# adaly/gridnext

Hardware: AMD Instinct MI355X
Metric: spots/sec training throughput (multimodal f+g) (higher is better)
Workload: dtype f32; 1 GPU; C4: multimodal f(DenseNet-121 @128px + count-MLP 2000 genes) + hex g on 78x64 Visium grids, 1 array (4992 spots) per GPU per step, f frozen/eval (tutorial mode), g trained with Adam, masked CE; spots_per_array=4992, parallelism=dp1

## Files before the change

gridnext_amd/csrc/stem_pool.hip:

```cpp
#include <type_traits>
#include "fwd_common.h"

namespace {

__global__ __launch_bounds__(256) void u8_to_f32_kernel(const uint8_t* __restrict__ x8, float* __restrict__ out, long n4,
                                                        long hw4, int C, const float* __restrict__ nrm) {
    const long stride = (long)gridDim.x * blockDim.x;
    for (long i = (long)blockIdx.x * blockDim.x + threadIdx.x; i < n4; i += stride) {
        const int c = (int)((i / hw4) % C);
        const bool norm = nrm != nullptr && c < 3;
        const float mean = norm ? nrm[c] : 0.f, sd = norm ? nrm[3 + c] : 1.f, rsd = norm ? nrm[6 + c] : 1.f;
        const uint32_t wv = reinterpret_cast<const uint32_t*>(x8)[i];
        reinterpret_cast<float4*>(out)[i] = u8x4_pixels(wv, norm, mean, sd, rsd);
    }
}

constexpr int ST_BM = 128, ST_BN = 64;

__global__ __launch_bounds__(256) void conv_stem_kernel(const float* __restrict__ x, const float* __restrict__ w,
                                                        float* __restrict__ out, long ldc, long M, int Cin, int H,
                                                        int Wd, int Ho, int Wo, int O, int KH, int KW, int stride,
                                                        int pad) {
    extern __shared__ __attribute__((aligned(16))) float lds[];
    const int KC = KH * 8, LD = KC + 4;
// ... 11 lines not shown
#pragma unroll
    for (int p = 0; p < 4; ++p) {
        const long row = m0 + rr + 32 * p;
        rok[p] = row < M;
        const long img = row / ((long)Ho * Wo);
        const int rem = (int)(row - img * Ho * Wo);
        const int oy = rem / Wo, ox = rem - oy * Wo;
        ibase[p] = img * Cin * (long)H * Wd;
        iy0[p] = oy * stride - pad;
        ix0[p] = ox * stride - pad + kx;
    }
    f32x16 acc[2];
#pragma unroll
    for (int a = 0; a < 2; ++a)
#pragma unroll
        for (int r = 0; r < 16; ++r) acc[a][r] = 0.f;

    for (int c = 0; c < Cin; ++c) {
        __syncthreads();
#pragma unroll
        for (int p = 0; p < 4; ++p) {
            const bool xok = rok[p] && kx < KW && ix0[p] >= 0 && ix0[p] < Wd;
            const float* xc = x + ibase[p] + (long)c * H * Wd;
            for (int ky = 0; ky < KH; ++ky) {
                const int iy = iy0[p] + ky;
                float v = 0.f;
                if (xok && iy >= 0 && iy < H) v = xc[(long)iy * Wd + ix0[p]];
                As[(rr + 32 * p) * LD + ky * 8 + kx] = v;
            }
        }
#pragma unroll
        for (int p = 0; p < 2; ++p) {
            const int o = n0 + rr + 32 * p;
            for (int ky = 0; ky < KH; ++ky) {
                float v = 0.f;
                if (o < O && kx < KW) v = w[(((long)o * Cin + c) * KH + ky) * KW + kx];
                Bs[(rr + 32 * p) * LD + ky * 8 + kx] = v;
            }
        }
        __syncthreads();
        for (int s = 0; s < KH; ++s) {
            const float4 a0 = ld4(&As[(64 * wm + i) * LD + 8 * s + 4 * h]);
            const float4 a1 = ld4(&As[(64 * wm + 32 + i) * LD + 8 * s + 4 * h]);
            const float4 b = ld4(&Bs[(32 * wn + i) * LD + 8 * s + 4 * h]);
            acc[0] = __builtin_amdgcn_mfma_f32_32x32x2f32(a0.x, b.x, acc[0], 0, 0, 0);
            acc[1] = __builtin_amdgcn_mfma_f32_32x32x2f32(a1.x, b.x, acc[1], 0, 0, 0);
            acc[0] = __builtin_amdgcn_mfma_f32_32x32x2f32(a0.y, b.y, acc[0], 0, 0, 0);
            acc[1] = __builtin_amdgcn_mfma_f32_32x32x2f32(a1.y, b.y, acc[1], 0, 0, 0);
            acc[0] = __builtin_amdgcn_mfma_f32_32x32x2f32(a0.z, b.z, acc[0], 0, 0, 0);
            acc[1] = __builtin_amdgcn_mfma_f32_32x32x2f32(a1.z, b.z, acc[1], 0, 0, 0);
            acc[0] = __builtin_amdgcn_mfma_f32_32x32x2f32(a0.w, b.w, acc[0], 0, 0, 0);
            acc[1] = __builtin_amdgcn_mfma_f32_32x32x2f32(a1.w, b.w, acc[1], 0, 0, 0);
        }
    }
    const int col = n0 + 32 * wn + i;
    if (col < O) {
#pragma unroll
        for (int mt = 0; mt < 2; ++mt)
#pragma unroll
            for (int r = 0; r < 16; ++r) {
                const long row = m0 + 64 * wm + 32 * mt + (r & 3) + 8 * (r >> 2) + 4 * h;
                if (row < M) out[row * ldc + col] = acc[mt][r];
            }
    }
}

template <int STRIDE, int KH, int CIN>
__global__ __launch_bounds__(256) void conv_stem_patch_kernel(const float* __restrict__ x, const float* __restrict__ w,
                                                              float* __restrict__ out, long ldc, int Cin, int H, int Wd,
                                                              int Ho, int Wo, int O, int KW, int pad, int tiles_x,
                                                              int tiles_y, long ntiles) {
    extern __shared__ __attribute__((aligned(16))) float lds[];
    constexpr int PH = 7 * STRIDE + KH, PW = (15 * STRIDE + 8 + 1) & ~1;
    const int KT = Cin * KH * 8, LDB = KT + 4;
    float* Bs = lds;
    float* Ps = lds + 64 * LDB;
    const int t = threadIdx.x, lane = t & 63, wave = t >> 6, h = lane >> 5, i = lane & 31;
    for (int idx = t; idx < 64 * KT; idx += 256) {
        const int n = idx / KT, rem = idx - n * KT;
        const int kx = rem & 7, cky = rem >> 3;
        float v = 0.f;
        if (n < O && kx < KW) v = w[((long)n * Cin * KH + cky) * KW + kx];
        Bs[n * LDB + rem] = v;
    }
    const int trow = 32 * wave + i;
    const int oyl = trow >> 4, oxl = trow & 15;
    const float* pa = Ps + (STRIDE * oyl) * PW + STRIDE * oxl + 4 * h;
    const float* pb = Bs + i * LDB + 4 * h;

    for (long tile = blockIdx.x; tile < ntiles; tile += gridDim.x) {
        const long img = tile / ((long)tiles_x * tiles_y);
        const int trem = (int)(tile - img * tiles_x * tiles_y);
        const int ty = trem / tiles_x, tx = trem - ty * tiles_x;
        const int oy0 = ty * 8, ox0 = tx * 16;
        const int iy0 = oy0 * STRIDE - pad, ix0 = ox0 * STRIDE - pad;
        __syncthreads();
        for (int idx = t; idx < Cin * PH * PW; idx += 256) {
            const int px = idx % PW, py = (idx / PW) % PH, c = idx / (PW * PH);
            const int iy = iy0 + py, ix = ix0 + px;
            float v = 0.f;
            if (iy >= 0 && iy < H && ix >= 0 && ix < Wd) v = x[((img * Cin + c) * H + iy) * (long)Wd + ix];
            Ps[idx] = v;
        }
        __syncthreads();
        f32x16 acc0, acc1;
#pragma unroll
        for (int r = 0; r < 16; ++r) { acc0[r] = 0.f; acc1[r] = 0.f; }
        auto load_a = [&](int step) {
            const float* ap = pa + ((step / KH) * PH + (step % KH)) * PW;
            if (STRIDE % 2 == 0) {
                const float2 lo = *reinterpret_cast<const float2*>(ap);
                const float2 hi = *reinterpret_cast<const float2*>(ap + 2);
                return make_float4(lo.x, lo.y, hi.x, hi.y);
            }
            return make_float4(ap[0], ap[1], ap[2], ap[3]);
        };
        constexpr int NSTEP = CIN * KH;
        float4 a = load_a(0), b0 = ld4(pb), b1 = ld4(pb + 32 * LDB);
#pragma unroll
        for (int step = 0; step < NSTEP; ++step) {
            float4 na = a, nb0 = b0, nb1 = b1;
            if (step + 1 < NSTEP) {
                na = load_a(step + 1);
                nb0 = ld4(pb + (step + 1) * 8);
                nb1 = ld4(pb + 32 * LDB + (step + 1) * 8);
            }
            acc0 = __builtin_amdgcn_mfma_f32_32x32x2f32(a.x, b0.x, acc0, 0, 0, 0);
            acc1 = __builtin_amdgcn_mfma_f32_32x32x2f32(a.x, b1.x, acc1, 0, 0, 0);
            acc0 = __builtin_amdgcn_mfma_f32_32x32x2f32(a.y, b0.y, acc0, 0, 0, 0);
            acc1 = __builtin_amdgcn_mfma_f32_32x32x2f32(a.y, b1.y, acc1, 0, 0, 0);
            acc0 = __builtin_amdgcn_mfma_f32_32x32x2f32(a.z, b0.z, acc0, 0, 0, 0);
            acc1 = __builtin_amdgcn_mfma_f32_32x32x2f32(a.z, b1.z, acc1, 0, 0, 0);
            acc0 = __builtin_amdgcn_mfma_f32_32x32x2f32(a.w, b0.w, acc0, 0, 0, 0);
            acc1 = __builtin_amdgcn_mfma_f32_32x32x2f32(a.w, b1.w, acc1, 0, 0, 0);
            a = na; b0 = nb0; b1 = nb1;
            __builtin_amdgcn_sched_group_barrier(0x100, STRIDE % 2 == 0 ? 4 : 6, 0);
            __builtin_amdgcn_sched_group_barrier(0x008, 8, 0);
        }
#pragma unroll
        for (int r = 0; r < 16; ++r) {
            const int rr = 32 * wave + (r & 3) + 8 * (r >> 2) + 4 * h;
            const int oy = oy0 + (rr >> 4), ox = ox0 + (rr & 15);
            if (oy < Ho && ox < Wo) {
                float* o = out + ((img * Ho + oy) * (long)Wo + ox) * ldc;
                if (i < O) o[i] = acc0[r];
                if (32 + i < O) o[32 + i] = acc1[r];
            }
        }
    }
}

constexpr int SP_LDT = 40;
constexpr int SP_LDTH = 72;
template <int WO, bool H16 = false, bool U8 = false, bool IDX = false>
__global__ __launch_bounds__(256) void conv_stem_pool_kernel(const void* __restrict__ xv, const float* __restrict__ w,
                                                             float* __restrict__ out, long ldo, int H, int Wd, int O,
                                                             const float* __restrict__ scale,
                                                             const float* __restrict__ shift, long imgs,
                                                             const float* __restrict__ nrm,
                                                             unsigned char* __restrict__ amax = nullptr,
                                                             const int* __restrict__ src_idx = nullptr, long src_imgs = 0) {
    const float* __restrict__ x = reinterpret_cast<const float*>(xv);
    const uint8_t* __restrict__ x8 = reinterpret_cast<const uint8_t*>(xv);
    constexpr int CIN = 3, KH = 7, KW = 7, STRIDE = 2, PAD = 3;
    constexpr int RT = 128 / WO;
    constexpr int PH = STRIDE * (RT - 1) + KH, PW = ((WO - 1) * STRIDE + 8 + 1 + 1) & ~1;
    constexpr int F4R = WO * STRIDE / 4;
    constexpr int NPC = CIN * PH * F4R, NPRE = (NPC + 255) / 256;
    constexpr int NIT = (WO / 2) * 8 / 256;
    constexpr int KT = CIN * KH * 8, LDB = KT + 4;
    extern __shared__ __attribute__((aligned(16))) float lds[];
    auto store4 = [](float* o, long off, const float4& v) {
        if constexpr (H16) {
            typedef _Float16 half4 __attribute__((ext_vector_type(4)));
            const half4 hv = {(_Float16)v.x, (_Float16)v.y, (_Float16)v.z, (_Float16)v.w};
            *reinterpret_cast<half4*>(reinterpret_cast<_Float16*>(o) + off) = hv;
        } else {
            *reinterpret_cast<float4*>(o + off) = v;
        }
    };
    float* Bs = lds;
    float* Ps = lds + 64 * LDB;
    float* Ts = Ps + CIN * PH * PW;
    const int t = threadIdx.x, lane = t & 63, wave = t >> 6, h = lane >> 5, i = lane & 31;
    for (int idx = t; idx < 64 * KT; idx += 256) {
        const int n = idx / KT, rem = idx - n * KT;
        const int kx = rem & 7, cky = rem >> 3;
        float v = 0.f;
        if (n < O && kx < KW) v = w[((long)n * CIN * KH + cky) * KW + kx];
        Bs[n * LDB + rem] = v;
    }
    for (int idx = t; idx < CIN * PH * PW; idx += 256) Ps[idx] = 0.f;
    const int trow = 32 * wave + i;
    const float* pa = Ps + (STRIDE * (trow / WO)) * PW + STRIDE * (trow % WO) + 4 * h;
    const float* pb = Bs + i * LDB + 4 * h;
    const float sc0 = i < O ? scale[i] : 0.f, sh0 = i < O ? shift[i] : 0.f;
    const float sc1 = 32 + i < O ? scale[32 + i] : 0.f, sh1 = 32 + i < O ? shift[32 + i] : 0.f;
    const int c4 = t & 7, pxa = t >> 3;
    const int Ho2 = (H + 2 * PAD - KH) / STRIDE + 1;
    const int ntt = Ho2 / RT;

    float4 pre[U8 ? 1 : NPRE];
    uint32_t pre8[U8 ? NPRE : 1];
    bool in8[U8 ? NPRE : 1];
    auto fetch_patch = [&](long img, int tt) {
        const int iy0 = RT * tt * STRIDE - PAD;
#pragma unroll
        for (int q = 0; q < NPRE; ++q) {
            const int j = t + 256 * q;
            const int f4 = j % F4R, py = (j / F4R) % PH, c = (j / F4R) / PH;
            const int iy = iy0 + py;
            const bool inside = j < NPC && iy >= 0 && iy < H;
            if constexpr (U8) {
                pre8[q] = 0u;
                in8[q] = inside;
                if (inside)
                    pre8[q] = *reinterpret_cast<const uint32_t*>(x8 + ((img * CIN + c) * H + iy) * (long)Wd + 4 * f4);
            } else {
                pre[q] = make_float4(0.f, 0.f, 0.f, 0.f);
                if (inside) pre[q] = ld4(x + ((img * CIN + c) * H + iy) * (long)Wd + 4 * f4);
            }
        }
    };
    auto stash_patch = [&]() {
#pragma unroll
        for (int q = 0; q < NPRE; ++q) {
            const int j = t + 256 * q;
            if (j < NPC) {
                float* d = Ps + (j / F4R) * PW + PAD + 4 * (j % F4R);
                if constexpr (U8) {
                    const int c = (j / F4R) / PH;
                    const bool norm = nrm != nullptr;
                    const float4 v = in8[q] ? u8x4_pixels(pre8[q], norm, norm ? nrm[c] : 0.f, norm ? nrm[3 + c] : 1.f,
                                                          norm ? nrm[6 + c] : 1.f)
                                            : make_float4(0.f, 0.f, 0.f, 0.f);
                    d[0] = v.x; d[1] = v.y; d[2] = v.z; d[3] = v.w;
                } else {
                    d[0] = pre[q].x; d[1] = pre[q].y; d[2] = pre[q].z; d[3] = pre[q].w;
                }
            }
        }
    };
    auto src_of = [&](long img) -> long {
        if (src_idx == nullptr) return img;
        const long s = src_idx[img];
        return s < 0 ? 0 : (s < src_imgs ? s : src_imgs - 1);
    };
    __syncthreads();
    fetch_patch(src_of(blockIdx.x), 0);

    for (long img = blockIdx.x; img < imgs; img += gridDim.x) {
        const long src = src_of(img);
        float4 carry[2][NIT], carry2[2][NIT];
        unsigned cidx[2][NIT], cidx2[2][NIT];
        const float c0v = IDX ? -1.f : 0.f;
#pragma unroll
        for (int q = 0; q < NIT; ++q) {
            carry[0][q] = carry[1][q] = carry2[0][q] = carry2[1][q] = make_float4(c0v, c0v, c0v, c0v);
            cidx[0][q] = cidx[1][q] = cidx2[0][q] = cidx2[1][q] = 0u;
        }
        for (int tt = 0; tt < ntt; ++tt) {
            __syncthreads();
            stash_patch();
            {
                long nsrc = src;
                int nt2 = tt + 1;
                if (nt2 == ntt) {
                    nt2 = 0;
                    long nimg = img + gridDim.x;
                    if (nimg >= imgs) nimg = blockIdx.x;
                    nsrc = src_of(nimg);
                }
                fetch_patch(nsrc, nt2);
            }
            asm volatile("" ::: "memory");
            __syncthreads();
            f32x16 acc0, acc1;
#pragma unroll
            for (int r = 0; r < 16; ++r) { acc0[r] = 0.f; acc1[r] = 0.f; }
            auto load_a = [&](int step) {
                const float* ap = pa + ((step / KH) * PH + (step % KH)) * PW;
                const float2 lo = *reinterpret_cast<const float2*>(ap);
                const float2 hi = *reinterpret_cast<const float2*>(ap + 2);
                return make_float4(lo.x, lo.y, hi.x, hi.y);
            };
            constexpr int NSTEP = CIN * KH;
            float4 a = load_a(0), b0 = ld4(pb), b1 = ld4(pb + 32 * LDB);
#pragma unroll
            for (int step = 0; step < NSTEP; ++step) {
                float4 na = a, nb0 = b0, nb1 = b1;
                if (step + 1 < NSTEP) {
                    na = load_a(step + 1);
                    nb0 = ld4(pb + (step + 1) * 8);
                    nb1 = ld4(pb + 32 * LDB + (step + 1) * 8);
                }
                acc0 = __builtin_amdgcn_mfma_f32_32x32x2f32(a.x, b0.x, acc0, 0, 0, 0);
                acc1 = __builtin_amdgcn_mfma_f32_32x32x2f32(a.x, b1.x, acc1, 0, 0, 0);
                acc0 = __builtin_amdgcn_mfma_f32_32x32x2f32(a.y, b0.y, acc0, 0, 0, 0);
                acc1 = __builtin_amdgcn_mfma_f32_32x32x2f32(a.y, b1.y, acc1, 0, 0, 0);
                acc0 = __builtin_amdgcn_mfma_f32_32x32x2f32(a.z, b0.z, acc0, 0, 0, 0);
                acc1 = __builtin_amdgcn_mfma_f32_32x32x2f32(a.z, b1.z, acc1, 0, 0, 0);
                acc0 = __builtin_amdgcn_mfma_f32_32x32x2f32(a.w, b0.w, acc0, 0, 0, 0);
                acc1 = __builtin_amdgcn_mfma_f32_32x32x2f32(a.w, b1.w, acc1, 0, 0, 0);
                a = na; b0 = nb0; b1 = nb1;
                __builtin_amdgcn_sched_group_barrier(0x100, 4, 0);
                __builtin_amdgcn_sched_group_barrier(0x008, 8, 0);
            }
#pragma unroll
            for (int pass = 0; pass < 2; ++pass) {
                if (pass == 1) __syncthreads();
#pragma unroll
                for (int r = 0; r < 16; ++r) {
                    const int rr = 32 * wave + (r & 3) + 8 * (r >> 2) + 4 * h;
                    Ts[rr * SP_LDT + i] = pass == 0 ? fmaxf(fmaf(acc0[r], sc0, sh0), 0.f) : fmaxf(fmaf(acc1[r], sc1, sh1), 0.f);
                }
                __syncthreads();
                const int ch = 32 * pass + 4 * c4;
#pragma unroll
                for (int q = 0; q < NIT; ++q) {
                    const int px = pxa + 32 * q;
                    float4 m0 = make_float4(c0v, c0v, c0v, c0v), m1 = m0;
                    unsigned h0 = 0u, h1 = 0u;
                    auto hmax = [](float4& m, unsigned& hx, const float4& v, unsigned col) {
                        if (IDX) {
                            if (v.x > m.x) { m.x = v.x; hx = (hx & 0xffffff00u) | col; }
                            if (v.y > m.y) { m.y = v.y; hx = (hx & 0xffff00ffu) | (col << 8); }
                            if (v.z > m.z) { m.z = v.z; hx = (hx & 0xff00ffffu) | (col << 16); }
                            if (v.w > m.w) { m.w = v.w; hx = (hx & 0x00ffffffu) | (col << 24); }
                        } else {
                            m = make_float4(fmaxf(m.x, v.x), fmaxf(m.y, v.y), fmaxf(m.z, v.z), fmaxf(m.w, v.w));
                        }
                    };
#pragma unroll
                    for (int dx = -1; dx <= 1; ++dx) {
                        const int ox = 2 * px + dx;
                        if (ox < 0) continue;
                        hmax(m0, h0, ld4(&Ts[ox * SP_LDT + 4 * c4]), (unsigned)(dx + 1));
                        if (RT == 2) hmax(m1, h1, ld4(&Ts[(WO + ox) * SP_LDT + 4 * c4]), (unsigned)(dx + 1));
                    }
                    auto vmax = [](const float4& ra, unsigned ia, const float4& rb, unsigned ib, const float4& rc, unsigned ic,
                                   float4& o4, unsigned& oi) {
                        if (IDX) {
                            o4 = ra; oi = ia;
                            const unsigned jb = ib + 0x03030303u, jc = ic + 0x06060606u;
                            if (rb.x > o4.x) { o4.x = rb.x; oi = (oi & 0xffffff00u) | (jb & 0x000000ffu); }
                            if (rb.y > o4.y) { o4.y = rb.y; oi = (oi & 0xffff00ffu) | (jb & 0x0000ff00u); }
                            if (rb.z > o4.z) { o4.z = rb.z; oi = (oi & 0xff00ffffu) | (jb & 0x00ff0000u); }
                            if (rb.w > o4.w) { o4.w = rb.w; oi = (oi & 0x00ffffffu) | (jb & 0xff000000u); }
                            if (rc.x > o4.x) { o4.x = rc.x; oi = (oi & 0xffffff00u) | (jc & 0x000000ffu); }
                            if (rc.y > o4.y) { o4.y = rc.y; oi = (oi & 0xffff00ffu) | (jc & 0x0000ff00u); }
                            if (rc.z > o4.z) { o4.z = rc.z; oi = (oi & 0xff00ffffu) | (jc & 0x00ff0000u); }
                            if (rc.w > o4.w) { o4.w = rc.w; oi = (oi & 0x00ffffffu) | (jc & 0xff000000u); }
                        } else {
                            o4 = make_float4(fmaxf(fmaxf(ra.x, rb.x), rc.x), fmaxf(fmaxf(ra.y, rb.y), rc.y),
                                             fmaxf(fmaxf(ra.z, rb.z), rc.z), fmaxf(fmaxf(ra.w, rb.w), rc.w));
                        }
                    };
                    if (RT == 2) {
                        float4 o4;
                        unsigned oi = 0u;
                        vmax(carry[pass][q], cidx[pass][q], m0, h0, m1, h1, o4, oi);
                        carry[pass][q] = m1;
                        cidx[pass][q] = h1;
                        if (ch < O) {
                            const long prow = (img * (Ho2 / 2) + tt) * (long)(WO / 2) + px;
                            store4(out, prow * ldo + ch, o4);
                            if (IDX) *reinterpret_cast<unsigned*>(amax + prow * O + ch) = oi;
                        }
                    } else {
                        if (tt & 1) {
                            float4 o4;
                            unsigned oi = 0u;
                            vmax(carry2[pass][q], cidx2[pass][q], carry[pass][q], cidx[pass][q], m0, h0, o4, oi);
                            if (ch < O) {
                                const long prow = (img * (Ho2 / 2) + (tt >> 1)) * (long)(WO / 2) + px;
                                store4(out, prow * ldo + ch, o4);
                                if (IDX) *reinterpret_cast<unsigned*>(amax + prow * O + ch) = oi;
                            }
                        }
                        carry2[pass][q] = carry[pass][q];
                        cidx2[pass][q] = cidx[pass][q];
                        carry[pass][q] = m0;
                        cidx[pass][q] = h0;
                    }
                }
            }
        }
    }
}

typedef _Float16 sp_half8 __attribute__((ext_vector_type(8)));
typedef _Float16 sp_half4 __attribute__((ext_vector_type(4)));
template <int WO, bool U8>
__global__ __launch_bounds__(256) void conv_stem_pool_f16_kernel(const void* __restrict__ xv, const float* __restrict__ w,
                                                                 _Float16* __restrict__ out, long ldo, int H, int Wd, int O,
                                                                 const float* __restrict__ scale,
                                                                 const float* __restrict__ shift, long imgs,
                                                                 const float* __restrict__ nrm, long obs = 32) {
    const float* __restrict__ x = reinterpret_cast<const float*>(xv);
    const uint8_t* __restrict__ x8 = reinterpret_cast<const uint8_t*>(xv);
    constexpr int CIN = 3, KH = 7, KW = 7, STRIDE = 2, PAD = 3;
    constexpr int RT = 128 / WO;
    constexpr int PH = 2 * RT + 5, NEW = STRIDE * RT, NV = RT == 1 ? 3 : 2;
    constexpr int PW = (WO - 1) * STRIDE + 8;
    constexpr int F4R = WO * STRIDE / 4;
    constexpr int NPC = CIN * NEW * F4R, NPRE = (NPC + 255) / 256;
    constexpr int NIT = (WO / 2) * 16 / 256;
    constexpr int NG = CIN * KH, NSTEP = (NG + 1) / 2;
    constexpr int LDBH = NSTEP * 16 + 8;
    extern __shared__ __attribute__((aligned(16))) float lds[];
    _Float16* Bs = reinterpret_cast<_Float16*>(lds);
    _Float16* Ps = Bs + 64 * LDBH;
    _Float16* Ts = Ps + ((CIN * PH * PW + 7) & ~7);
    const int t = threadIdx.x, lane = t & 63, wave = t >> 6, h = lane >> 5, i = lane & 31;
    for (int idx = t; idx < 64 * LDBH; idx += 256) {
        const int n = idx / LDBH, rem = idx - n * LDBH;
        const int kx = rem & 7, cky = rem >> 3;
        float v = 0.f;
        if (n < O && kx < KW && cky < NG) v = w[((long)n * CIN * KH + cky) * KW + kx];
        Bs[idx] = (_Float16)v;
    }
    for (int idx = t; idx < CIN * PH * PW; idx += 256) Ps[idx] = (_Float16)0.f;
    const int trow = 32 * wave + i;
    const _Float16* pa = Ps + STRIDE * (trow % WO);
    const int rr2 = STRIDE * (trow / WO);
    const _Float16* pb = Bs + i * LDBH + 8 * h;
    const float sc0 = i < O ? scale[i] : 0.f, sh0 = i < O ? shift[i] : 0.f;
    const float sc1 = 32 + i < O ? scale[32 + i] : 0.f, sh1 = 32 + i < O ? shift[32 + i] : 0.f;
    const int c4 = t & 15, pxa = t >> 4;
    const int Ho2 = (H + 2 * PAD - KH) / STRIDE + 1;
    const int ntt = Ho2 / RT;

    float4 pre[U8 ? 1 : NPRE];
    uint32_t pre8[U8 ? NPRE : 1];
    bool in8[U8 ? NPRE : 1];
    auto fetch_patch = [&](long img, int tt) {
        const int iy0 = NEW * tt + 2;
#pragma unroll
        for (int q = 0; q < NPRE; ++q) {
            const int j = t + 256 * q;
            const int f4 = j % F4R, py = (j / F4R) % NEW, c = (j / F4R) / NEW;
            const int iy = iy0 + py;
            const bool inside = j < NPC && iy >= 0 && iy < H;
            if constexpr (U8) {
                pre8[q] = 0u;
                in8[q] = inside;
                if (inside)
                    pre8[q] = *reinterpret_cast<const uint32_t*>(x8 + ((img * CIN + c) * H + iy) * (long)Wd + 4 * f4);
            } else {
                pre[q] = make_float4(0.f, 0.f, 0.f, 0.f);
                if (inside) pre[q] = ld4(x + ((img * CIN + c) * H + iy) * (long)Wd + 4 * f4);
            }
        }
    };
    auto stash_patch = [&](int tt) {
#pragma unroll
        for (int q = 0; q < NPRE; ++q) {
            const int j = t + 256 * q;
            if (j < NPC) {
// ... 122 lines not shown
                                                             const float* __restrict__ shift,
                                                             unsigned char* __restrict__ amax) {
    const long total = Mout * C;
    for (long idx = (long)blockIdx.x * blockDim.x + threadIdx.x; idx < total; idx += (long)gridDim.x * blockDim.x) {
        const long row = idx / C;
        const int c = (int)(idx - row * C);
        const long img = row / ((long)Ho * Wo);
        const int rem = (int)(row - img * Ho * Wo);
        const int oy = rem / Wo, ox = rem - oy * Wo;
        const float sc = scale[c], sh = shift[c];
        float m = IDX ? -1.f : 0.f;
        int am = 0;
#pragma unroll
        for (int dy = -1; dy <= 1; ++dy) {
            const int iy = 2 * oy + dy;
            if (iy < 0 || iy >= Hi) continue;
#pragma unroll
            for (int dx = -1; dx <= 1; ++dx) {
                const int ix = 2 * ox + dx;
                if (ix < 0 || ix >= Wi) continue;
                const float v = fmaxf(fmaf(in[((img * Hi + iy) * Wi + ix) * ldi + c], sc, sh), 0.f);
                if (IDX) { if (v > m) { m = v; am = 3 * (dy + 1) + dx + 1; } }
                else m = fmaxf(m, v);
            }
        }
        out[row * ldo + c] = m;
        if (IDX) amax[row * C + c] = (unsigned char)am;
    }
}

template <bool IDX>
__global__ __launch_bounds__(256) void bnrelu_maxpool_vec4_kernel(const float* __restrict__ in, long ldi,
                                                                  float* __restrict__ out, long ldo, long Mout, int C4,
                                                                  int Hi, int Wi, int Ho, int Wo,
                                                                  const float* __restrict__ scale,
                                                                  const float* __restrict__ shift,
                                                                  unsigned char* __restrict__ amax) {
    const long total = Mout * C4;
    for (long idx = (long)blockIdx.x * blockDim.x + threadIdx.x; idx < total; idx += (long)gridDim.x * blockDim.x) {
        const long row = idx / C4;
        const int c = 4 * (int)(idx - row * C4);
        const long img = row / ((long)Ho * Wo);
        const int rem = (int)(row - img * Ho * Wo);
        const int oy = rem / Wo, ox = rem - oy * Wo;
        const float4 sc = ld4(scale + c), sh = ld4(shift + c);
        const float m0 = IDX ? -1.f : 0.f;
        float4 m = make_float4(m0, m0, m0, m0);
        unsigned am = 0;
#pragma unroll
        for (int dy = -1; dy <= 1; ++dy) {
            const int iy = 2 * oy + dy;
            if (iy < 0 || iy >= Hi) continue;
#pragma unroll
            for (int dx = -1; dx <= 1; ++dx) {
                const int ix = 2 * ox + dx;
                if (ix < 0 || ix >= Wi) continue;
                const float4 v = ld4(in + ((img * Hi + iy) * Wi + ix) * ldi + c);
                const float a0 = fmaxf(fmaf(v.x, sc.x, sh.x), 0.f), a1 = fmaxf(fmaf(v.y, sc.y, sh.y), 0.f);
                const float a2 = fmaxf(fmaf(v.z, sc.z, sh.z), 0.f), a3 = fmaxf(fmaf(v.w, sc.w, sh.w), 0.f);
                if (IDX) {
                    const unsigned li = 3 * (dy + 1) + dx + 1;
                    if (a0 > m.x) { m.x = a0; am = (am & 0xffffff00u) | li; }
                    if (a1 > m.y) { m.y = a1; am = (am & 0xffff00ffu) | (li << 8); }
                    if (a2 > m.z) { m.z = a2; am = (am & 0xff00ffffu) | (li << 16); }
                    if (a3 > m.w) { m.w = a3; am = (am & 0x00ffffffu) | (li << 24); }
                } else {
                    m.x = fmaxf(m.x, a0); m.y = fmaxf(m.y, a1); m.z = fmaxf(m.z, a2); m.w = fmaxf(m.w, a3);
                }
            }
        }
        *reinterpret_cast<float4*>(out + row * ldo + c) = m;
        if (IDX) *reinterpret_cast<unsigned*>(amax + row * (4L * C4) + c) = am;
    }
}

template <bool IN16 = false>
__global__ __launch_bounds__(256) void bnrelu_avgpool_kernel(const float* __restrict__ in, long ldi, float* __restrict__ out,
                                                             long ldo, int C, int S2, const float* __restrict__ scale,
                                                             const float* __restrict__ shift, long ibs = 32,
                                                             const int* __restrict__ dst_idx = nullptr, long dst_rows = 0) {
    __shared__ float red[4][64];
    const int cl = threadIdx.x & 63, rl = threadIdx.x >> 6;
    const int c = blockIdx.y * 64 + cl;
    const long img = blockIdx.x;
    float acc = 0.f;
    if (c < C) {
        const float sc = scale[c], sh = shift[c];
        for (int r = rl; r < S2; r += 4) {
            const long off = (img * S2 + r) * ldi + (c >> 5) * ibs + (c & 31);
            const float v = IN16 ? (float)reinterpret_cast<const _Float16*>(in)[off] : in[off];
            acc += fmaxf(fmaf(v, sc, sh), 0.f);
        }
    }
    red[rl][cl] = acc;
    __syncthreads();
    if (rl == 0 && c < C) {
        long orow = img;
        if (dst_idx != nullptr) {
            orow = dst_idx[img];
            if (orow < 0 || orow >= dst_rows) return;
        }
        out[orow * ldo + c] = ((red[0][cl] + red[1][cl]) + (red[2][cl] + red[3][cl])) / (float)S2;
    }
}

}

GNX_EXPORT int gnx_conv_stem(const float* x, const float* w, float* out, long ldc, long imgs, int Cin, int H, int W,
                             int O, int KH, int KW, int stride, int pad, hipStream_t stream) {
    if (!x || !w || !out || imgs < 0 || Cin <= 0 || O <= 0 || KH <= 0 || KH > 7 || KW <= 0 || KW > 8 || stride <= 0 ||
        ldc < O)
        return GNX_ERR_BAD_ARG;
    const int Ho = (H + 2 * pad - KH) / stride + 1, Wo = (W + 2 * pad - KW) / stride + 1;
    if (Ho <= 0 || Wo <= 0) return GNX_ERR_BAD_ARG;
    const long M = imgs * Ho * Wo;
    if (M == 0) return GNX_OK;
    if (O <= 64 && Cin == 3 && ((stride == 2 && KH == 7 && KW == 7) || (stride == 1 && KH == 3 && KW == 3))) {
        const int tiles_x = gnx_cdiv(Wo, 16), tiles_y = gnx_cdiv(Ho, 8);
        const long ntiles = imgs * tiles_x * tiles_y;
        const int PH = 7 * stride + KH, PW = (15 * stride + 8 + 1) & ~1;
        const size_t lds2 = ((size_t)64 * (Cin * KH * 8 + 4) + (size_t)Cin * PH * PW) * sizeof(float);
        const int grid2 = (int)(ntiles < 256 * 3 ? ntiles : 256 * 3);
        if (stride == 2)
            conv_stem_patch_kernel<2, 7, 3><<<grid2, 256, lds2, stream>>>(x, w, out, ldc, Cin, H, W, Ho, Wo, O, KW, pad,
                                                                      tiles_x, tiles_y, ntiles);
        else
            conv_stem_patch_kernel<1, 3, 3><<<grid2, 256, lds2, stream>>>(x, w, out, ldc, Cin, H, W, Ho, Wo, O, KW, pad,
                                                                      tiles_x, tiles_y, ntiles);
        return gnx_launch_status();
    }
    const size_t lds_bytes = (size_t)(ST_BM + ST_BN) * (KH * 8 + 4) * sizeof(float);
    dim3 grid(gnx_cdiv(M, ST_BM), gnx_cdiv(O, ST_BN));
    conv_stem_kernel<<<grid, 256, lds_bytes, stream>>>(x, w, out, ldc, M, Cin, H, W, Ho, Wo, O, KH, KW, stride, pad);
    return gnx_launch_status();
}

template <bool H16, bool U8 = false>
static int stem_pool_launch(const void* x, const float* w, float* out, long ldo, long imgs, int Cin, int H, int W, int O,
                            int KH, int KW, int stride, int pad, const float* scale, const float* shift, hipStream_t stream,
                            const float* nrm = nullptr, unsigned char* amax = nullptr, const int* src_idx = nullptr,
                            long src_imgs = 0) {
    if (!x || !w || !out || !scale || !shift || imgs < 0 || Cin <= 0 || O <= 0 || H <= 0 || W <= 0 || ldo < O)
        return GNX_ERR_BAD_ARG;
    if (src_idx && (src_imgs <= 0 || amax)) return GNX_ERR_BAD_ARG;
    if (amax && (H16 || U8 || (reinterpret_cast<uintptr_t>(amax) & 3) != 0)) return GNX_ERR_UNSUPPORTED;
    if (Cin != 3 || KH != 7 || KW != 7 || stride != 2 || pad != 3 || O > 64 || O % 4 != 0 || ldo % 4 != 0 ||
        (reinterpret_cast<uintptr_t>(out) & (H16 ? 7 : 15)) != 0)
        return GNX_ERR_UNSUPPORTED;
    const int Ho = (H + 6 - 7) / 2 + 1, Wo = (W + 6 - 7) / 2 + 1;
    if ((Wo != 64 && Wo != 128) || W != 2 * Wo || Ho % 2 != 0 || Ho <= 0 ||
        (reinterpret_cast<uintptr_t>(x) & (U8 ? 3 : 15)) != 0)
        return GNX_ERR_UNSUPPORTED;
    if (imgs == 0) return GNX_OK;
    const int RT = 128 / Wo, PH = 2 * (RT - 1) + 7, PW = ((Wo - 1) * 2 + 8 + 2) & ~1;
    const size_t lds_bytes = ((size_t)64 * (3 * 7 * 8 + 4) + (size_t)3 * PH * PW + (size_t)128 * SP_LDT) * sizeof(float);
    const int per_cu = lds_bytes <= 80 * 1024 ? 2 : 1;
    const int grid = (int)(imgs < 256 * per_cu ? imgs : 256 * per_cu);
    if (Wo == 64) {
        static bool conf = false;
        if (!conf) {
            if (hipFuncSetAttribute(reinterpret_cast<const void*>(conv_stem_pool_kernel<64, H16, U8>),
                                    hipFuncAttributeMaxDynamicSharedMemorySize, (int)lds_bytes) != hipSuccess)
                return GNX_ERR_LAUNCH;
            conf = true;
        }
        if constexpr (!H16 && !U8) {
            if (amax) {
                static bool confi = false;
                if (!confi) {
                    if (hipFuncSetAttribute(reinterpret_cast<const void*>(conv_stem_pool_kernel<64, false, false, true>),
                                            hipFuncAttributeMaxDynamicSharedMemorySize, (int)lds_bytes) != hipSuccess)
                        return GNX_ERR_LAUNCH;
                    confi = true;
                }
                conv_stem_pool_kernel<64, false, false, true><<<grid, 256, lds_bytes, stream>>>(x, w, out, ldo, H, W, O, scale,
                                                                                                shift, imgs, nrm, amax);
                return gnx_launch_status();
            }
        }
        conv_stem_pool_kernel<64, H16, U8><<<grid, 256, lds_bytes, stream>>>(x, w, out, ldo, H, W, O, scale, shift, imgs, nrm,
                                                                             nullptr, src_idx, src_imgs);
    } else {
        static bool conf = false;
        if (!conf) {
            if (hipFuncSetAttribute(reinterpret_cast<const void*>(conv_stem_pool_kernel<128, H16, U8>),
                                    hipFuncAttributeMaxDynamicSharedMemorySize, (int)lds_bytes) != hipSuccess)
                return GNX_ERR_LAUNCH;
            conf = true;
        }
        if constexpr (!H16 && !U8) {
            if (amax) {
                static bool confi = false;
                if (!confi) {
                    if (hipFuncSetAttribute(reinterpret_cast<const void*>(conv_stem_pool_kernel<128, false, false, true>),
                                            hipFuncAttributeMaxDynamicSharedMemorySize, (int)lds_bytes) != hipSuccess)
                        return GNX_ERR_LAUNCH;
                    confi = true;
                }
                conv_stem_pool_kernel<128, false, false, true><<<grid, 256, lds_bytes, stream>>>(x, w, out, ldo, H, W, O, scale,
                                                                                                 shift, imgs, nrm, amax);
                return gnx_launch_status();
            }
        }
        conv_stem_pool_kernel<128, H16, U8><<<grid, 256, lds_bytes, stream>>>(x, w, out, ldo, H, W, O, scale, shift, imgs, nrm,
                                                                              nullptr, src_idx, src_imgs);
    }
    return gnx_launch_status();
}
GNX_EXPORT int gnx_conv_stem_bnrelu_maxpool(const float* x, const float* w, float* out, long ldo, long imgs, int Cin,
                                            int H, int W, int O, int KH, int KW, int stride, int pad, const float* scale,
                                            const float* shift, hipStream_t stream) {
    return stem_pool_launch<false>(x, w, out, ldo, imgs, Cin, H, W, O, KH, KW, stride, pad, scale, shift, stream);
}
GNX_EXPORT int gnx_conv_stem_bnrelu_maxpool_idx(const float* x, const float* w, float* out, long ldo, long imgs, int Cin,
                                                int H, int W, int O, int KH, int KW, int stride, int pad, const float* scale,
                                                const float* shift, const int* src_idx, long src_imgs, hipStream_t stream) {
    if (!src_idx) return GNX_ERR_BAD_ARG;
    return stem_pool_launch<false>(x, w, out, ldo, imgs, Cin, H, W, O, KH, KW, stride, pad, scale, shift, stream, nullptr,
                                   nullptr, src_idx, src_imgs);
}
GNX_EXPORT int gnx_conv_stem_bnrelu_maxpool_argmax(const float* x, const float* w, float* out, long ldo,
                                                   unsigned char* argmax, long imgs, int Cin, int H, int W, int O, int KH,
                                                   int KW, int stride, int pad, const float* scale, const float* shift,
                                                   hipStream_t stream) {
    if (!argmax) return GNX_ERR_BAD_ARG;
    return stem_pool_launch<false>(x, w, out, ldo, imgs, Cin, H, W, O, KH, KW, stride, pad, scale, shift, stream, nullptr,
                                   argmax);
}
GNX_EXPORT int gnx_conv_stem_bnrelu_maxpool_h16(const float* x, const float* w, void* out16, long ldo, long imgs, int Cin,
                                                int H, int W, int O, int KH, int KW, int stride, int pad,
                                                const float* scale, const float* shift, hipStream_t stream) {
    return stem_pool_launch<true>(x, w, reinterpret_cast<float*>(out16), ldo, imgs, Cin, H, W, O, KH, KW, stride, pad, scale,
                                  shift, stream);
}

template <bool U8>
static int stem_pool_f16_launch(const void* x, const float* w, void* out16, long ldo, long imgs, int Cin, int H, int W, int O,
                                int KH, int KW, int stride, int pad, const float* scale, const float* shift,
                                const float* nrm, hipStream_t stream, long obs = 32) {
    if (!x || !w || !out16 || !scale || !shift || imgs < 0 || Cin <= 0 || O <= 0 || H <= 0 || W <= 0 ||
        (obs == 32 ? ldo < O : ldo != 32))
        return GNX_ERR_BAD_ARG;
    if (Cin != 3 || KH != 7 || KW != 7 || stride != 2 || pad != 3 || O > 64 || O % 4 != 0 || ldo % 4 != 0 ||
        (reinterpret_cast<uintptr_t>(out16) & 7) != 0)
        return GNX_ERR_UNSUPPORTED;
    const int Ho = (H + 6 - 7) / 2 + 1, Wo = (W + 6 - 7) / 2 + 1;
    if ((Wo != 64 && Wo != 128) || W != 2 * Wo || Ho % 2 != 0 || Ho <= 0 ||
        (reinterpret_cast<uintptr_t>(x) & (U8 ? 3 : 15)) != 0)
        return GNX_ERR_UNSUPPORTED;
    if (imgs == 0) return GNX_OK;
    const int RT = 128 / Wo, PH = 2 * RT + 5, PW = (Wo - 1) * 2 + 8;
    const size_t lds_bytes = ((size_t)64 * (11 * 16 + 8) + (size_t)((3 * PH * PW + 7) & ~7) + (size_t)128 * SP_LDTH) * 2;
    const int per_cu = lds_bytes <= 53 * 1024 ? 3 : 2;
    const int grid = (int)(imgs < 256 * per_cu ? imgs : 256 * per_cu);
    _Float16* o = reinterpret_cast<_Float16*>(out16);
    if (Wo == 64)
        conv_stem_pool_f16_kernel<64, U8><<<grid, 256, lds_bytes, stream>>>(x, w, o, ldo, H, W, O, scale, shift, imgs, nrm, obs);
    else
        conv_stem_pool_f16_kernel<128, U8><<<grid, 256, lds_bytes, stream>>>(x, w, o, ldo, H, W, O, scale, shift, imgs, nrm, obs);
    return gnx_launch_status();
}
GNX_EXPORT int gnx_conv_stem_bnrelu_maxpool_f16mul(const void* x, int x_is_u8, const float* w, void* out16, long ldo,
                                                   long imgs, int Cin, int H, int W, int O, int KH, int KW, int stride,
                                                   int pad, const float* scale, const float* shift, const float* norm,
                                                   hipStream_t stream) {
    if (x_is_u8)
        return stem_pool_f16_launch<true>(x, w, out16, ldo, imgs, Cin, H, W, O, KH, KW, stride, pad, scale, shift, norm, stream);
    if (norm) return GNX_ERR_BAD_ARG;
    return stem_pool_f16_launch<false>(x, w, out16, ldo, imgs, Cin, H, W, O, KH, KW, stride, pad, scale, shift, nullptr, stream);
}
GNX_EXPORT int gnx_conv_stem_bnrelu_maxpool_f16mul_cb(const void* x, int x_is_u8, const float* w, void* out16, long rows_total,
                                                      long imgs, int Cin, int H, int W, int O, int KH, int KW, int stride,
                                                      int pad, const float* scale, const float* shift, const float* norm,
                                                      hipStream_t stream) {
    if (rows_total <= 0 || O % 32 != 0) return GNX_ERR_BAD_ARG;
    if (imgs > 0 && H > 0 && W > 0) {
        const long hp = ((H - 1) / 2 + 1) / 2, wp = ((W - 1) / 2 + 1) / 2;
        if (hp > 0 && wp > 0 && rows_total / (hp * wp) < imgs) return GNX_ERR_BAD_ARG;
    }
    if (x_is_u8)
        return stem_pool_f16_launch<true>(x, w, out16, 32, imgs, Cin, H, W, O, KH, KW, stride, pad, scale, shift, norm, stream,
                                          rows_total * 32);
    if (norm) return GNX_ERR_BAD_ARG;
    return stem_pool_f16_launch<false>(x, w, out16, 32, imgs, Cin, H, W, O, KH, KW, stride, pad, scale, shift, nullptr, stream,
                                       rows_total * 32);
}

GNX_EXPORT int gnx_conv_stem_bnrelu_maxpool_u8(const uint8_t* x8, const float* w, void* out, long ldo, long imgs, int Cin,
                                               int H, int W, int O, int KH, int KW, int stride, int pad, const float* scale,
                                               const float* shift, const float* norm, int out_f16, hipStream_t stream) {
    if (out_f16)
        return stem_pool_launch<true, true>(x8, w, reinterpret_cast<float*>(out), ldo, imgs, Cin, H, W, O, KH, KW, stride, pad,
                                            scale, shift, stream, norm);
    return stem_pool_launch<false, true>(x8, w, reinterpret_cast<float*>(out), ldo, imgs, Cin, H, W, O, KH, KW, stride, pad,
                                         scale, shift, stream, norm);
}

GNX_EXPORT int gnx_conv_stem_bnrelu_maxpool_u8_idx(const uint8_t* x8, const float* w, float* out, long ldo, long imgs, int Cin,
                                                   int H, int W, int O, int KH, int KW, int stride, int pad, const float* scale,
                                                   const float* shift, const float* norm, const int* src_idx, long src_imgs,
                                                   hipStream_t stream) {
    if (!src_idx) return GNX_ERR_BAD_ARG;
    return stem_pool_launch<false, true>(x8, w, out, ldo, imgs, Cin, H, W, O, KH, KW, stride, pad, scale, shift, stream, norm,
                                         nullptr, src_idx, src_imgs);
}

GNX_EXPORT int gnx_u8_to_f32(const uint8_t* x8, float* out, long imgs, int C, int H, int W, const float* norm,
                             hipStream_t stream) {
// ... 90 lines not shown
```

Baseline: 88930 spots/s.

## Use ring-buffered input rows and dense tap packing in fused stem conv-pool

The fused 7x7 stride-2 stem conv+maxpool kernel now keeps a ring buffer of input rows in LDS. Each output tile fetches only the new rows instead of reloading the whole overlapping window, and the first tiles of each image prime the ring. The K dimension is also repacked from 3x7x8 padded taps (168 with zero padding) to the 147 real taps paired for the 32x32x2 MFMA, which removes the wasted multiply-accumulates on padding. The price is a switch over ring base offsets that compiles several unrolled variants, extra warm-up iterations per image, and scalar A loads that replace float4 loads.

```diff
diff --git a/gridnext_amd/csrc/stem_pool.hip b/gridnext_amd/csrc/stem_pool.hip
--- a/gridnext_amd/csrc/stem_pool.hip
+++ b/gridnext_amd/csrc/stem_pool.hip
@@ -187,6 +187,25 @@
 
 constexpr int SP_LDT = 40;
 constexpr int SP_LDTH = 72;
+constexpr int SP_NTAP = 3 * 7 * 7, SP_NMUL = (SP_NTAP + 1) / 2;
+constexpr int SP_BH = (SP_NMUL + 3) & ~3;
+constexpr int SP_LDB = 2 * SP_BH + 4;
+__host__ __device__ constexpr int sp_tap_group(int q) { return q / 7; }
+__host__ __device__ constexpr int sp_tap_kx(int q) { return (q % 7) & 1 ? 4 + (q % 7) / 2 : (q % 7) / 2; }
+template <int PHR, int PW, int B>
+__host__ __device__ constexpr int sp_ring_off(int q) {
+    return q < SP_NTAP ? ((sp_tap_group(q) / 7) * PHR + (B + sp_tap_group(q) % 7) % PHR) * PW + sp_tap_kx(q)
+                       : sp_ring_off<PHR, PW, B>(q - 1) + 4;
+}
+template <int PHR, int PW, int B>
+__host__ __device__ constexpr bool sp_ring_distances_ok() {
+    const int dch = sp_ring_off<PHR, PW, B>(49) - sp_ring_off<PHR, PW, B>(48);
+    for (int p = 0; p < SP_NMUL; ++p) {
+        const int d = sp_ring_off<PHR, PW, B>(2 * p + 1) - sp_ring_off<PHR, PW, B>(2 * p);
+        if (d != 4 && d != -3 && d != PW - 3 && d != (1 - PHR) * PW - 3 && d != dch) return false;
+    }
+    return true;
+}
 template <int WO, bool H16 = false, bool U8 = false, bool IDX = false>
 __global__ __launch_bounds__(256) void conv_stem_pool_kernel(const void* __restrict__ xv, const float* __restrict__ w,
                                                              float* __restrict__ out, long ldo, int H, int Wd, int O,
@@ -199,11 +218,14 @@
     const uint8_t* __restrict__ x8 = reinterpret_cast<const uint8_t*>(xv);
     constexpr int CIN = 3, KH = 7, KW = 7, STRIDE = 2, PAD = 3;
     constexpr int RT = 128 / WO;
-    constexpr int PH = STRIDE * (RT - 1) + KH, PW = ((WO - 1) * STRIDE + 8 + 1 + 1) & ~1;
+    constexpr int NEW = STRIDE * RT, NV = RT == 1 ? 3 : 2;
+    constexpr int PH = RT == 1 ? 8 : 12, PW = ((WO - 1) * STRIDE + 8 + 1 + 1) & ~1;
+    static_assert(PH % NEW == 0 && PH >= STRIDE * (RT - 1) + KH, "the ring holds a tile's window");
     constexpr int F4R = WO * STRIDE / 4;
-    constexpr int NPC = CIN * PH * F4R, NPRE = (NPC + 255) / 256;
+    constexpr int NPC = CIN * NEW * F4R, NPRE = (NPC + 255) / 256;
     constexpr int NIT = (WO / 2) * 8 / 256;
-    constexpr int KT = CIN * KH * 8, LDB = KT + 4;
+    constexpr int LDB = SP_LDB;
+    static_assert(CIN * KH * KW == SP_NTAP, "the tap sequence is written for 3 x 7 x 7");
     extern __shared__ __attribute__((aligned(16))) float lds[];
     auto store4 = [](float* o, long off, const float4& v) {
         if constexpr (H16) {
@@ -218,17 +240,18 @@
     float* Ps = lds + 64 * LDB;
     float* Ts = Ps + CIN * PH * PW;
     const int t = threadIdx.x, lane = t & 63, wave = t >> 6, h = lane >> 5, i = lane & 31;
-    for (int idx = t; idx < 64 * KT; idx += 256) {
-        const int n = idx / KT, rem = idx - n * KT;
-        const int kx = rem & 7, cky = rem >> 3;
+    for (int idx = t; idx < 64 * 2 * SP_BH; idx += 256) {
+        const int n = idx / (2 * SP_BH), rem = idx - n * (2 * SP_BH);
+        const int hh = rem / SP_BH, p = rem - hh * SP_BH, q = 2 * p + hh;
         float v = 0.f;
-        if (n < O && kx < KW) v = w[((long)n * CIN * KH + cky) * KW + kx];
+        if (n < O && q < SP_NTAP) v = w[((long)n * CIN * KH + sp_tap_group(q)) * KW + sp_tap_kx(q)];
         Bs[n * LDB + rem] = v;
     }
     for (int idx = t; idx < CIN * PH * PW; idx += 256) Ps[idx] = 0.f;
     const int trow = 32 * wave + i;
-    const float* pa = Ps + (STRIDE * (trow / WO)) * PW + STRIDE * (trow % WO) + 4 * h;
-    const float* pb = Bs + i * LDB + 4 * h;
+    const float* pa0 = Ps + STRIDE * (trow % WO);
+    const int rr2 = STRIDE * (trow / WO);
+    const float* pb = Bs + i * LDB + SP_BH * h;
     const float sc0 = i < O ? scale[i] : 0.f, sh0 = i < O ? shift[i] : 0.f;
     const float sc1 = 32 + i < O ? scale[32 + i] : 0.f, sh1 = 32 + i < O ? shift[32 + i] : 0.f;
     const int c4 = t & 7, pxa = t >> 3;
@@ -239,11 +262,11 @@
     uint32_t pre8[U8 ? NPRE : 1];
     bool in8[U8 ? NPRE : 1];
     auto fetch_patch = [&](long img, int tt) {
-        const int iy0 = RT * tt * STRIDE - PAD;
+        const int iy0 = NEW * tt + 2;
 #pragma unroll
         for (int q = 0; q < NPRE; ++q) {
             const int j = t + 256 * q;
-            const int f4 = j % F4R, py = (j / F4R) % PH, c = (j / F4R) / PH;
+            const int f4 = j % F4R, py = (j / F4R) % NEW, c = (j / F4R) / NEW;
             const int iy = iy0 + py;
             const bool inside = j < NPC && iy >= 0 && iy < H;
             if constexpr (U8) {
@@ -257,14 +280,16 @@
             }
         }
     };
-    auto stash_patch = [&]() {
+    auto stash_patch = [&](int tt) {
 #pragma unroll
         for (int q = 0; q < NPRE; ++q) {
             const int j = t + 256 * q;
             if (j < NPC) {
-                float* d = Ps + (j / F4R) * PW + PAD + 4 * (j % F4R);
+                const int py = (j / F4R) % NEW, cc = (j / F4R) / NEW;
+                const int slot = (NEW * tt + 2 + py + PAD + PH) % PH;
+                float* d = Ps + (cc * PH + slot) * PW + PAD + 4 * (j % F4R);
                 if constexpr (U8) {
-                    const int c = (j / F4R) / PH;
+                    const int c = cc;
                     const bool norm = nrm != nullptr;
                     const float4 v = in8[q] ? u8x4_pixels(pre8[q], norm, norm ? nrm[c] : 0.f, norm ? nrm[3 + c] : 1.f,
                                                           norm ? nrm[6 + c] : 1.f)
@@ -282,7 +307,7 @@
         return s < 0 ? 0 : (s < src_imgs ? s : src_imgs - 1);
     };
     __syncthreads();
-    fetch_patch(src_of(blockIdx.x), 0);
+    fetch_patch(src_of(blockIdx.x), -NV);
 
     for (long img = blockIdx.x; img < imgs; img += gridDim.x) {
         const long src = src_of(img);
@@ -294,14 +319,14 @@
             carry[0][q] = carry[1][q] = carry2[0][q] = carry2[1][q] = make_float4(c0v, c0v, c0v, c0v);
             cidx[0][q] = cidx[1][q] = cidx2[0][q] = cidx2[1][q] = 0u;
         }
-        for (int tt = 0; tt < ntt; ++tt) {
+        for (int tt = -NV; tt < ntt; ++tt) {
             __syncthreads();
-            stash_patch();
+            stash_patch(tt);
             {
                 long nsrc = src;
                 int nt2 = tt + 1;
                 if (nt2 == ntt) {
-                    nt2 = 0;
+                    nt2 = -NV;
                     long nimg = img + gridDim.x;
                     if (nimg >= imgs) nimg = blockIdx.x;
                     nsrc = src_of(nimg);
@@ -309,37 +334,65 @@
                 fetch_patch(nsrc, nt2);
             }
             asm volatile("" ::: "memory");
+            if (tt < 0) continue;
             __syncthreads();
             f32x16 acc0, acc1;
 #pragma unroll
             for (int r = 0; r < 16; ++r) { acc0[r] = 0.f; acc1[r] = 0.f; }
-            auto load_a = [&](int step) {
-                const float* ap = pa + ((step / KH) * PH + (step % KH)) * PW;
-                const float2 lo = *reinterpret_cast<const float2*>(ap);
-                const float2 hi = *reinterpret_cast<const float2*>(ap + 2);
-                return make_float4(lo.x, lo.y, hi.x, hi.y);
+            const int base = __builtin_amdgcn_readfirstlane((NEW * tt + rr2) % PH);
+            auto multiply = [&](auto bc) {
+                constexpr int B = decltype(bc)::value;
+                static_assert(sp_ring_distances_ok<PH, PW, B>(), "a pair of taps without a base pointer");
+                constexpr int D_FWD = 4, D_BACK = -3, D_ROW = PW - 3, D_WRAP = (1 - PH) * PW - 3;
+                constexpr int D_CH = sp_ring_off<PH, PW, B>(49) - sp_ring_off<PH, PW, B>(48);
+                const float* pa_fwd = pa0 + D_FWD * h;
+                const float* pa_back = pa0 + D_BACK * h;
+                const float* pa_row = pa0 + D_ROW * h;
+                const float* pa_wrap = pa0 + D_WRAP * h;
+                const float* pa_ch = pa0 + D_CH * h;
+                auto load_a = [&](int p) {
+                    const int o0 = sp_ring_off<PH, PW, B>(2 * p), d = sp_ring_off<PH, PW, B>(2 * p + 1) - o0;
+                    const float* bp = d == D_FWD ? pa_fwd : d == D_BACK ? pa_back : d == D_ROW ? pa_row : d == D_WRAP ? pa_wrap : pa_ch;
+                    return bp[o0];
+                };
+                constexpr int NCHUNK = (SP_NMUL + 3) / 4;
+                float a[4], na[4];
+#pragma unroll
+                for (int k = 0; k < 4; ++k) a[k] = load_a(k);
+                float4 b0 = ld4(pb), b1 = ld4(pb + 32 * LDB);
+#pragma unroll
+                for (int ch = 0; ch < NCHUNK; ++ch) {
+                    float4 nb0 = b0, nb1 = b1;
+#pragma unroll
+                    for (int k = 0; k < 4; ++k) na[k] = a[k];
+                    if (ch + 1 < NCHUNK) {
+#pragma unroll
+                        for (int k = 0; k < 4; ++k)
+                            if (4 * (ch + 1) + k < SP_NMUL) na[k] = load_a(4 * (ch + 1) + k);
+                        nb0 = ld4(pb + 4 * (ch + 1));
+                        nb1 = ld4(pb + 32 * LDB + 4 * (ch + 1));
+                    }
+                    const float bv0[4] = {b0.x, b0.y, b0.z, b0.w}, bv1[4] = {b1.x, b1.y, b1.z, b1.w};
+#pragma unroll
+                    for (int k = 0; k < 4; ++k)
+                        if (4 * ch + k < SP_NMUL) {
+                            acc0 = __builtin_amdgcn_mfma_f32_32x32x2f32(a[k], bv0[k], acc0, 0, 0, 0);
+                            acc1 = __builtin_amdgcn_mfma_f32_32x32x2f32(a[k], bv1[k], acc1, 0, 0, 0);
+                        }
+#pragma unroll
+                    for (int k = 0; k < 4; ++k) a[k] = na[k];
+                    b0 = nb0; b1 = nb1;
+                    __builtin_amdgcn_sched_group_barrier(0x100, 6, 0);
+                    __builtin_amdgcn_sched_group_barrier(0x008, 8, 0);
+                }
             };
-            constexpr int NSTEP = CIN * KH;
-            float4 a = load_a(0), b0 = ld4(pb), b1 = ld4(pb + 32 * LDB);
-#pragma unroll
-            for (int step = 0; step < NSTEP; ++step) {
-                float4 na = a, nb0 = b0, nb1 = b1;
-                if (step + 1 < NSTEP) {
-                    na = load_a(step + 1);
-                    nb0 = ld4(pb + (step + 1) * 8);
-                    nb1 = ld4(pb + 32 * LDB + (step + 1) * 8);
-                }
-                acc0 = __builtin_amdgcn_mfma_f32_32x32x2f32(a.x, b0.x, acc0, 0, 0, 0);
-                acc1 = __builtin_amdgcn_mfma_f32_32x32x2f32(a.x, b1.x, acc1, 0, 0, 0);
-                acc0 = __builtin_amdgcn_mfma_f32_32x32x2f32(a.y, b0.y, acc0, 0, 0, 0);
-                acc1 = __builtin_amdgcn_mfma_f32_32x32x2f32(a.y, b1.y, acc1, 0, 0, 0);
-                acc0 = __builtin_amdgcn_mfma_f32_32x32x2f32(a.z, b0.z, acc0, 0, 0, 0);
-                acc1 = __builtin_amdgcn_mfma_f32_32x32x2f32(a.z, b1.z, acc1, 0, 0, 0);
-                acc0 = __builtin_amdgcn_mfma_f32_32x32x2f32(a.w, b0.w, acc0, 0, 0, 0);
-                acc1 = __builtin_amdgcn_mfma_f32_32x32x2f32(a.w, b1.w, acc1, 0, 0, 0);
-                a = na; b0 = nb0; b1 = nb1;
-                __builtin_amdgcn_sched_group_barrier(0x100, 4, 0);
-                __builtin_amdgcn_sched_group_barrier(0x008, 8, 0);
+            switch (base) {
+                case 0: multiply(std::integral_constant<int, 0>{}); break;
+                case 2: multiply(std::integral_constant<int, 2>{}); break;
+                case 4: multiply(std::integral_constant<int, 4>{}); break;
+                case 6: multiply(std::integral_constant<int, 6>{}); break;
+                case 8: multiply(std::integral_constant<int, 8 % PH>{}); break;
+                default: multiply(std::integral_constant<int, 10 % PH>{}); break;
             }
 #pragma unroll
             for (int pass = 0; pass < 2; ++pass) {
@@ -768,8 +821,8 @@
         (reinterpret_cast<uintptr_t>(x) & (U8 ? 3 : 15)) != 0)
         return GNX_ERR_UNSUPPORTED;
     if (imgs == 0) return GNX_OK;
-    const int RT = 128 / Wo, PH = 2 * (RT - 1) + 7, PW = ((Wo - 1) * 2 + 8 + 2) & ~1;
-    const size_t lds_bytes = ((size_t)64 * (3 * 7 * 8 + 4) + (size_t)3 * PH * PW + (size_t)128 * SP_LDT) * sizeof(float);
+    const int RT = 128 / Wo, PH = RT == 1 ? 8 : 12, PW = ((Wo - 1) * 2 + 8 + 2) & ~1;
+    const size_t lds_bytes = ((size_t)64 * SP_LDB + (size_t)3 * PH * PW + (size_t)128 * SP_LDT) * sizeof(float);
     const int per_cu = lds_bytes <= 80 * 1024 ? 2 : 1;
     const int grid = (int)(imgs < 256 * per_cu ? imgs : 256 * per_cu);
     if (Wo == 64) {
```

Result: no change. 88980 spots/s, median of 2 (+0.1%).
